# jspenmar/slowtv_monodepth

Measured on AMD Instinct MI355X. Metric: training images/sec (640×192, 3-frame) at 1/2/4/8 MI355X; warp+SSIM HBM GB/s, higher is better.
Workload: dtype f32

## Files before the change

include/smd_hotpath.h:

```cpp
#ifndef SMD_HOTPATH_H
#define SMD_HOTPATH_H

#include <stddef.h>
#include <stdint.h>

#ifdef __cplusplus
extern "C" {
#endif

#define SMD_ABI_VERSION 8

#define SMD_OK 0
#define SMD_E_INVALID (-1)
#define SMD_E_LAUNCH (-2)
#define SMD_E_WORKSPACE (-3)
#define SMD_E_UNSUPPORTED (-4)

#define SMD_USE_MIN 0x1
#define SMD_USE_AUTOMASK 0x2
#define SMD_LOSS_L1 0x4
#define SMD_NEED_K_GRAD 0x8
#define SMD_USE_EDGES 0x10
#define SMD_LOSS_L2 0x20
#define SMD_MASK_EXPLAINABILITY 0x80
// ... 151 lines not shown
int smd_conv3x3_mfma_fwd(const void* xp, const void* wp_fwd, void* y, void* workspace, size_t workspace_bytes,
                         int B, int C, int CO, int h, int w, int pieces, void* stream);
int smd_conv3x3_mfma_bwd_data(const void* g_y, const void* wp_bwd, void* g_xp, void* workspace, size_t workspace_bytes,
                              int B, int C, int CO, int h, int w, int pieces, void* stream);
int smd_conv3x3_mfma_bwd_weight(const void* xp, const void* g_y, float* g_weight, void* workspace, size_t workspace_bytes,
                                int B, int C, int CO, int h, int w, int pieces, void* stream);

size_t smd_conv3x3z_mfma_workspace_bytes(int B, int C, int CO, int h, int w);
int smd_conv3x3z_mfma_fwd(const float* x, const void* wp_fwd, float* y, void* workspace, size_t workspace_bytes,
                          int B, int C, int CO, int h, int w, int pieces, void* stream);
int smd_conv3x3z_mfma_bwd_data(const float* g_y, const void* wp_bwd, float* g_x, void* workspace, size_t workspace_bytes,
                               int B, int C, int CO, int h, int w, int pieces, void* stream);
int smd_conv3x3z_mfma_bwd_weight(const float* x, const float* g_y, float* g_weight, void* workspace, size_t workspace_bytes,
                                 int B, int C, int CO, int h, int w, int pieces, void* stream);

size_t smd_conv7x7s2_packed_bytes(int C, int CO);
size_t smd_conv7x7s2_workspace_bytes(int B, int C, int CO, int H, int W);
int smd_conv7x7s2_pack(const float* weight, void* wp, int C, int CO, void* stream);
int smd_conv7x7s2_fwd(const float* x, const void* wp, float* y, int B, int C, int CO, int H, int W, void* stream);
int smd_conv7x7s2_bwd_weight(const float* x, const float* g_y, float* g_weight, void* workspace, size_t workspace_bytes,
                             int B, int C, int CO, int H, int W, void* stream);

size_t smd_bn_workspace_bytes(int N, int C, int HW);
int smd_bn_fwd(const float* x, const float* residual, const float* gamma, const float* beta, float* running_mean, float* running_var,
               float momentum, float eps, int relu, float* y, float* save_mean, float* save_invstd,
               void* workspace, size_t workspace_bytes, int N, int C, int HW, void* stream);
int smd_bn_bwd(const float* x, const float* y, const float* g_y, const float* gamma, const float* save_mean, const float* save_invstd,
               int relu, float* g_x, float* g_residual, float* g_gamma, float* g_beta,
               void* workspace, size_t workspace_bytes, int N, int C, int HW, void* stream);

// ... 98 lines not shown
```

slowtv_monodepth_amd/_lib.py:

```python
from __future__ import annotations

import ctypes as C
import os
from pathlib import Path

import torch

__all__ = ['lib', 'call', 'set_knob', 'reset_knobs', 'knob_epoch', 'lib_path', 'FLAGS', 'REGR_FLAGS', 'SEL_MASKED', 'ptr_array', 'int_array', 'i64_array', 'HotpathError', 'Unsupported']

_HERE = Path(__file__).resolve().parent
lib_path = Path(os.environ.get('SMD_HOTPATH_LIB', _HERE/'libsmd_hotpath.so'))

FLAGS = {'use_min': 0x1, 'use_automask': 0x2, 'loss_l1': 0x4, 'need_k_grad': 0x8, 'use_edges': 0x10, 'loss_l2': 0x20, 'packed_ready': 0x40,
         'mask_explainability': 0x80, 'mask_uncertainty': 0x100, 'use_laplacian': 0x200, 'bwd_skip_rows': 0x400, 'edges_ready': 0x800, 'bwd_no_live': 0x1000}
REGR_FLAGS = {'l1': 0x0, 'log_l1': 0x1, 'berhu': 0x2, 'invert': 0x4}
SEL_MASKED = 255
MAX_SCALES = 8
MAX_SUPPORTS = 8

_vp, _i, _f, _sz, _u64 = C.c_void_p, C.c_int, C.c_float, C.c_size_t, C.c_uint64

PROTOTYPES = {
    'smd_last_error': (C.c_char_p, []),
    'smd_abi_version': (_i, []),
# ... 46 lines not shown
    'smd_scale_mean_fwd': (_i, [_vp]*2 + [_i]*2 + [_vp]*2 + [_sz, _vp]),
    'smd_scale_mean_bwd': (_i, [_vp]*2 + [_i]*2 + [_vp]*3),
    'smd_conv3x3_thin_workspace_bytes': (_sz, [_i]*4),
    'smd_conv3x3_thin_fwd': (_i, [_vp]*3 + [_i]*4 + [_vp]),
    'smd_conv3x3_thin_bwd': (_i, [_vp]*6 + [_sz] + [_i]*4 + [_vp]),
    'smd_conv3x3_mfma_packed_bytes': (_sz, [_i]*3),
    'smd_conv3x3_mfma_workspace_bytes': (_sz, [_i]*5),
    'smd_conv3x3_mfma_pack': (_i, [_vp]*3 + [_i]*3 + [_vp]),
    'smd_conv3x3_mfma_fwd': (_i, [_vp]*4 + [_sz] + [_i]*6 + [_vp]),
    'smd_conv3x3_mfma_bwd_data': (_i, [_vp]*4 + [_sz] + [_i]*6 + [_vp]),
    'smd_conv3x3_mfma_bwd_weight': (_i, [_vp]*4 + [_sz] + [_i]*6 + [_vp]),
    'smd_conv3x3z_mfma_workspace_bytes': (_sz, [_i]*5),
    'smd_conv3x3z_mfma_fwd': (_i, [_vp]*4 + [_sz] + [_i]*6 + [_vp]),
    'smd_conv3x3z_mfma_bwd_data': (_i, [_vp]*4 + [_sz] + [_i]*6 + [_vp]),
    'smd_conv3x3z_mfma_bwd_weight': (_i, [_vp]*4 + [_sz] + [_i]*6 + [_vp]),
    'smd_conv7x7s2_packed_bytes': (_sz, [_i]*2),
    'smd_conv7x7s2_workspace_bytes': (_sz, [_i]*5),
    'smd_conv7x7s2_pack': (_i, [_vp]*2 + [_i]*2 + [_vp]),
    'smd_conv7x7s2_fwd': (_i, [_vp]*3 + [_i]*5 + [_vp]),
    'smd_conv7x7s2_bwd_weight': (_i, [_vp]*4 + [_sz] + [_i]*5 + [_vp]),
    'smd_conv3x3_head_workspace_bytes': (_sz, [_i]*4),
    'smd_conv3x3_head_fwd': (_i, [_vp]*4 + [_i]*5 + [_vp]),
    'smd_conv3x3_head_bwd': (_i, [_vp]*8 + [_sz] + [_i]*5 + [_vp]),
    'smd_elu_pad_fwd': (_i, [_vp]*3 + [_i]*6 + [_vp]),
    'smd_elu_pad_bwd': (_i, [_vp]*6 + [_sz] + [_i]*6 + [_vp]),
    'smd_elu_up_cat_pad_fwd': (_i, [_vp]*4 + [_i]*6 + [_vp]),
    'smd_elu_up_cat_pad_bwd': (_i, [_vp]*7 + [_sz] + [_i]*6 + [_vp]),
    'smd_bn_workspace_bytes': (_sz, [_i, _i, _i]),
    'smd_bn_fwd': (_i, [_vp]*6 + [_f, _f, _i] + [_vp]*4 + [_sz] + [_i]*3 + [_vp]),
    'smd_bn_bwd': (_i, [_vp]*6 + [_i] + [_vp]*5 + [_sz] + [_i]*3 + [_vp]),
# ... 102 lines not shown
```

slowtv_monodepth_amd/conv_ops.py:

```python
from __future__ import annotations

from collections import namedtuple

import torch

from . import _lib
from ._device import _check, _check_fb, _on, _ptr, _stream, _workspace, call
from .conv_routing import serve

_BF = torch.bfloat16


def _thin_bwd(xp, weight, g_y, want_x, want_w):
    if not (want_x or want_w): return None, None
    B, C, H, W = xp.shape
    g_xp = torch.empty_like(xp) if want_x else None
    g_w = torch.empty_like(weight) if want_w else None
    ws, nbytes = _workspace(xp.device, _lib.lib.smd_conv3x3_thin_workspace_bytes, B, C, H - 2, W - 2, floor=256) if want_w else (None, 0)
    call('smd_conv3x3_thin_bwd', xp.data_ptr(), weight.data_ptr(), g_y.data_ptr(), _ptr(g_xp), _ptr(g_w), _ptr(ws), nbytes, B, C, H - 2, W - 2, _stream())
    return g_xp, g_w


class _Conv3x3Thin(torch.autograd.Function):
    @staticmethod
# ... 38 lines not shown
    return wf, wb


def _mfma_ws_bytes(B, C, CO, h, w, zpad):
    return (_lib.lib.smd_conv3x3z_mfma_workspace_bytes if zpad else _lib.lib.smd_conv3x3_mfma_workspace_bytes)(B, C, CO, h, w)


def _mfma_launch(entry, zpad, a, b, out, nws, dims, pieces):
    ws, nws = _workspace(out.device, nws, floor=256)
    call(('smd_conv3x3z_mfma_' if zpad else 'smd_conv3x3_mfma_') + entry, a.data_ptr(), b.data_ptr(), out.data_ptr(), ws.data_ptr(), nws, *dims, pieces, _stream())
    return out


class _Conv3x3Wide(torch.autograd.Function):
    @staticmethod
    def forward(ctx, xp, weight, pieces, force, zpad=False):
        xp = _check_fb('xp', xp)
        if zpad and xp.dtype != torch.float32: raise TypeError(f'the zero-padded convolution takes float32 tensors, got {xp.dtype}')
        if xp.ndim != 4 or (not zpad and (xp.shape[2] < 3 or xp.shape[3] < 3)):
            raise ValueError(f'expected {"(B,C,h,w)" if zpad else "a padded (B,C,h+2,w+2)"}, got {tuple(xp.shape)}')
        B, C, H, W = xp.shape
        if weight.ndim != 4 or tuple(weight.shape[1:]) != (C, 3, 3): raise ValueError(f'weight: expected (CO,{C},3,3), got {tuple(weight.shape)}')
        CO = weight.shape[0]
        weight = _check('weight', weight, (CO, C, 3, 3))
        h, w = (H, W) if zpad else (H - 2, W - 2)
        dims = (B, C, CO, h, w)
        bf = xp.dtype == _BF
        if bf: pieces = 1
        nws = _mfma_ws_bytes(*dims, zpad)
        sv = _served(C, CO, zpad, force or nws > 0)
        if force and not sv.fwd:
# ... 6 lines not shown
            return _mfma_launch('fwd', zpad, xp, packed['wf'], y, nws, dims, pieces)

        def run_ref():
            if zpad: return torch.conv2d(xp, weight, None, 1, 1)
            if bf: return torch.conv2d(xp, weight.to(_BF))
            if sv.thin: call('smd_conv3x3_thin_fwd', xp.data_ptr(), weight.data_ptr(), y.data_ptr(), B, C, h, w, _stream()); return y
            return torch.conv2d(xp, weight)
        op = 'fwd_z' if zpad else 'fwd_bf16' if bf else 'fwd'
        out = serve((op, *dims), run_mfma, run_ref, eligible=sv.fwd and sv.sized, force=force)
        ctx.save_for_backward(xp, weight, packed.get('wb'))
        ctx.pieces, ctx.force, ctx.zpad, ctx.served = pieces, force, zpad, sv
        return out

    @staticmethod
    def backward(ctx, g_y):
        xp, weight, wp_bwd = ctx.saved_tensors
        return (*_wide_backward(xp, weight, wp_bwd, g_y, ctx.pieces, ctx.force, ctx.zpad, ctx.served, *ctx.needs_input_grad[:2]), None, None, None)


def _wide_backward(xp, weight, wp_bwd, g_y, pieces, force, zpad, sv, need_x, need_w, deterministic_ref=False):
    _on(xp)
    B, C, H, W = xp.shape
    CO = weight.shape[0]
    h, w = (H, W) if zpad else (H - 2, W - 2)
    dims = (B, C, CO, h, w)
    bf = xp.dtype == _BF
    g_y = _check_fb('grad(y)', g_y.to(xp.dtype), (B, CO, h, w))
    g_xp = g_w = None
    w_ref = weight.to(_BF) if bf else weight
    pad = [1, 1] if zpad else [0, 0]
    def cb(mask):
        det = torch.backends.cudnn.deterministic
# ... 20 lines not shown
    return g_xp, g_w


def conv3x3_mfma(xp, weight, pieces: int = 3):
    return _Conv3x3Wide.apply(xp, weight, int(pieces), True)


def conv3x3_wide(xp, weight):
    return _Conv3x3Wide.apply(xp, weight, 3, False)


def conv3x3_same(x, weight):
    return _Conv3x3Wide.apply(x, weight, 3, False, True)


class _Conv7x7s2Stem(torch.autograd.Function):
    @staticmethod
    def forward(ctx, x, weight):
        x = _check('x', x)
        if x.ndim != 4: raise ValueError(f'expected (B,C,H,W), got {tuple(x.shape)}')
        B, C, H, W = x.shape
        if weight.ndim != 4 or tuple(weight.shape[1:]) != (C, 7, 7): raise ValueError(f'weight: expected (CO,{C},7,7), got {tuple(weight.shape)}')
        CO = weight.shape[0]
        weight = _check('weight', weight, (CO, C, 7, 7))
        ho, wo = (H - 1)//2 + 1, (W - 1)//2 + 1
        served = _lib.lib.smd_conv7x7s2_workspace_bytes(B, C, CO, H, W) > 0
        y = torch.empty((B, CO, ho, wo), device=x.device, dtype=torch.float32)

        def run_mfma():
            wp, _ = _workspace(x.device, _lib.lib.smd_conv7x7s2_packed_bytes, C, CO)
# ... 33 lines not shown
```

slowtv_monodepth_amd/conv_routing.py:

```python
from __future__ import annotations

import torch

from ._lib import Unsupported

_MODE = 'auto'
_ROUTES: dict = {}
_AB_WARMUPS, _AB_ROUNDS, _AB_MARGIN = 2, 5, 0.97
_DECLINED = (Unsupported, ValueError)


def set_conv_route(mode: str = 'auto'):
    global _MODE
    if mode not in ('auto', 'mfma', 'miopen'): raise ValueError(mode)
    _MODE = mode
    _ROUTES.clear()


def conv_routes() -> dict:
    return dict(_ROUTES)


_COARSE_W_MAX, _COARSE_C_MIN = 80, 256
_Z_FWD_WGT = [dict(px_min=1000, ch_max=511), dict(px_min=2400)]
# ... 3 lines not shown
               'wgt': [dict(thin=False, px_min=20000, co_max=64), dict(thin=False, coarse=True, px_min=2400)]},
    'bf16': {'fwd': [dict(thin=True)], 'data': [dict(thin=True)], 'wgt': [dict(thin=True)]},
    'zpad': {'fwd': _Z_FWD_WGT, 'data': [dict(px_min=1000)], 'wgt': _Z_FWD_WGT},
    'stem': {'fwd': [dict(px_min=20000)], 'wgt': [dict(px_min=20000)]},
}
_FAMILY_OF_SUFFIX = {'': 'padded', 'bf16': 'bf16', 'z': 'zpad', 's': 'stem'}
_BOUNDS = {'px_min': lambda v, B, C, CO, h, w: B*h*w >= v,
           'c_max': lambda v, B, C, CO, h, w: C <= v,
           'co_max': lambda v, B, C, CO, h, w: CO <= v,
           'c_co_max': lambda v, B, C, CO, h, w: C*CO <= v,
           'ch_max': lambda v, B, C, CO, h, w: max(C, CO) <= v,
           'thin': lambda v, B, C, CO, h, w: (CO == 16) == v,
           'coarse': lambda v, B, C, CO, h, w: (w <= _COARSE_W_MAX and C >= _COARSE_C_MIN) == v}


def static_rule(op, B, C, CO, h, w) -> bool:
    kind, _, suffix = op.partition('_')
    clauses = STATIC_RULES[_FAMILY_OF_SUFFIX[suffix]][kind]
    return any(all(_BOUNDS[name](v, B, C, CO, h, w) for name, v in clause.items()) for clause in clauses)


_capturing = torch.cuda.is_current_stream_capturing


def _time_interleaved(run_mfma, run_ref, rounds):
    ev = [[torch.cuda.Event(enable_timing=True) for _ in range(3)] for _ in range(rounds)]
    for e in ev:
        e[0].record(); run_mfma(); e[1].record(); run_ref(); e[2].record()
    torch.cuda.synchronize()
    return [e[0].elapsed_time(e[1])*1e3 for e in ev], [e[1].elapsed_time(e[2])*1e3 for e in ev]


def _conv_route(op, B, C, CO, h, w, run_mfma, run_ref) -> bool:
    if _MODE != 'auto': return _MODE == 'mfma'
# ... 26 lines not shown
```

slowtv_monodepth_amd/csrc/smd_api.hip:

```cpp
#include <limits.h>
#include <math.h>
#include <stdarg.h>
#include <stdio.h>
#include <stdlib.h>
#include <string.h>
#include <algorithm>

#include "smd_kernels.h"
#include "smd_smooth_dev.h"

namespace {

thread_local char g_err[512] = "";

int fail(int code, const char* fmt, ...) {
  va_list ap;
  va_start(ap, fmt);
  vsnprintf(g_err, sizeof(g_err), fmt, ap);
  va_end(ap);
  return code;
}

int check_launch(hipError_t e, const char* what) {
  if (e != hipSuccess) return fail(SMD_E_LAUNCH, "%s: %s", what, hipGetErrorString(e));
// ... 880 lines not shown
int smd_conv3x3_mfma_bwd_data(const void* g_y, const void* wp_bwd, void* g_xp, void* workspace, size_t workspace_bytes, int B, int C, int CO, int h, int w, int pieces, void* stream) {
  return mfma_form(ConvOp::Data, false, g_y, wp_bwd, g_xp, workspace, workspace_bytes, B, C, CO, h, w, pieces, stream, "conv3x3_mfma_bwd_data");
}
int smd_conv3x3_mfma_bwd_weight(const void* xp, const void* g_y, float* g_weight, void* workspace, size_t workspace_bytes, int B, int C, int CO, int h, int w, int pieces, void* stream) {
  return mfma_bwd_weight(false, xp, g_y, g_weight, workspace, workspace_bytes, B, C, CO, h, w, pieces, stream);
}
int smd_conv3x3z_mfma_fwd(const float* x, const void* wp_fwd, float* y, void* workspace, size_t workspace_bytes, int B, int C, int CO, int h, int w, int pieces, void* stream) {
  return mfma_form(ConvOp::Fwd, true, x, wp_fwd, y, workspace, workspace_bytes, B, C, CO, h, w, pieces, stream, "conv3x3z_mfma_fwd");
}
int smd_conv3x3z_mfma_bwd_data(const float* g_y, const void* wp_bwd, float* g_x, void* workspace, size_t workspace_bytes, int B, int C, int CO, int h, int w, int pieces, void* stream) {
  return mfma_form(ConvOp::Data, true, g_y, wp_bwd, g_x, workspace, workspace_bytes, B, C, CO, h, w, pieces, stream, "conv3x3z_mfma_bwd_data");
}
int smd_conv3x3z_mfma_bwd_weight(const float* x, const float* g_y, float* g_weight, void* workspace, size_t workspace_bytes, int B, int C, int CO, int h, int w, int pieces, void* stream) {
  return mfma_bwd_weight(true, x, g_y, g_weight, workspace, workspace_bytes, B, C, CO, h, w, pieces, stream);
}
static bool stem_sizes_ok(int B, int C, int H, int W) {
  if (B < 1 || B > 65535 || C < 1 || H < 1 || W < 1) return false;
  const long long ho = (H - 1)/2 + 1, wo = (W - 1)/2 + 1;
  return (long long)C*H*W < (1ll << 31) && 64*ho*wo < (1ll << 31) && (ho + 3)/4 <= 65535;
}
size_t smd_conv7x7s2_packed_bytes(int C, int CO) { return smd::conv_stem_served(C, CO) ? smd::conv_stem_packed_bytes(C) : 0; }
size_t smd_conv7x7s2_workspace_bytes(int B, int C, int CO, int H, int W) {
  if (!smd::conv_stem_served(C, CO) || !stem_sizes_ok(B, C, H, W)) return 0;
  return align256(smd::conv_stem_wgrad_floats(B, C, H, W)*sizeof(float));
}
int smd_conv7x7s2_pack(const float* weight, void* wp, int C, int CO, void* stream) {
  if (!weight || !wp) return fail(SMD_E_INVALID, "null pointer");
  if (!smd::conv_stem_served(C, CO)) return fail(SMD_E_UNSUPPORTED, "the stem kernels serve CO == 64 with C == 3 | 6, not C=%d CO=%d", C, CO);
  return check_launch(smd::launch_conv_stem_pack(weight, wp, C, (hipStream_t)stream), "conv7x7s2_pack");
}
// ... 406 lines not shown
```

slowtv_monodepth_amd/csrc/smd_conv_mfma.hip:

```cpp
#include "smd_common.h"
#include "smd_kernels.h"
#include "smd_conv_mfma_dev.h"
#include <algorithm>

namespace smd {

template <typename T> __device__ __forceinline__ void store_out(T* p, size_t i, float v);
template <> __device__ __forceinline__ void store_out<float>(float* p, size_t i, float v) { p[i] = v; }
template <> __device__ __forceinline__ void store_out<bf16>(bf16* p, size_t i, float v) { p[i] = __float2bfloat16(v); }

template <int P>
__global__ __launch_bounds__(256) void k_conv_pack_w(const float* __restrict__ w, unsigned short* __restrict__ wp_fwd, unsigned short* __restrict__ wp_bwd, int CO, int C) {
  const int idx = blockIdx.x*256 + threadIdx.x;
  if (idx >= CO*C*9) return;
  const int tap = idx % 9, c = (idx/9) % C, co = idx/(9*C);
  unsigned pk[P];
  split_pair<P>(w[idx], 0.f, pk);
  if (wp_fwd) {
    const size_t base = ((((size_t)(co >> 5)*(C >> 4) + (c >> 4))*9 + tap)*P)*512 + (((c >> 3) & 1)*32 + (co & 31))*8 + (c & 7);
#pragma unroll
    for (int p = 0; p < P; ++p) wp_fwd[base + (size_t)p*512] = (unsigned short)(pk[p] & 0xffffu);
  }
  if (wp_bwd) {
    const size_t base = ((((size_t)(c >> 5)*(CO >> 4) + (co >> 4))*9 + (8 - tap))*P)*512 + (((co >> 3) & 1)*32 + (c & 31))*8 + (co & 7);
// ... 284 lines not shown
    }
  }
}

template <typename TO>
__global__ __launch_bounds__(256) void k_conv_split_sum(const float* __restrict__ part, TO* __restrict__ out, size_t n4, int KS) {
  const size_t i = (size_t)blockIdx.x*256 + threadIdx.x;
  if (i >= n4) return;
  const f4* p = reinterpret_cast<const f4*>(part);
  f4 s = p[i];
  for (int k = 1; k < KS; ++k) s += p[(size_t)k*n4 + i];
  if constexpr (sizeof(TO) == 4) reinterpret_cast<f4*>(out)[i] = s;
  else { unsigned* o = reinterpret_cast<unsigned*>(out) + 2*i; o[0] = pack_bf16_rne(s.x, s.y); o[1] = pack_bf16_rne(s.z, s.w); }
}

static size_t thin_packed_elems(int C, int pieces) { return (size_t)(C >> 4)*5*pieces*512; }
size_t conv_mfma_packed_elems(int C, int CO, int pieces) { return std::max((size_t)CO*C*9*pieces, CO == 16 ? thin_packed_elems(C, pieces) : (size_t)0); }

#define SMD_BY_PIECES(pieces, CALL) do { if ((pieces) == 3) { CALL(3, float); } else if ((pieces) == 2) { CALL(2, float); } else { CALL(1, bf16); } } while (0)

template <int P, typename T>
static void launch_conv16(const void* in, const void* wp, void* out, int B, int CK, bool bwd, int hi, int wi, int ho, int wo, hipStream_t st) {
  const unsigned gx = ceil_div(wo, 64), gy = ceil_div(ho, 4), gz = B;
  const dim3 grid(8*(unsigned)ceil_div((long long)gx*gy*gz, 8ll));
  const uint4* wq = (const uint4*)wp;
  const T* i_ = (const T*)in; T* o_ = (T*)out;
  if (bwd) hipLaunchKernelGGL((k_conv16_mfma<1, P, true, T, T>), grid, dim3(256), 0, st, i_, wq, o_, hi, wi, ho, wo, gx, gy, gz);
  else if (CK == 16) hipLaunchKernelGGL((k_conv16_mfma<1, P, false, T, T>), grid, dim3(256), 0, st, i_, wq, o_, hi, wi, ho, wo, gx, gy, gz);
  else hipLaunchKernelGGL((k_conv16_mfma<2, P, false, T, T>), grid, dim3(256), 0, st, i_, wq, o_, hi, wi, ho, wo, gx, gy, gz);
}
// ... 137 lines not shown
```

slowtv_monodepth_amd/csrc/smd_kernels.h:

```cpp
#pragma once
#include <hip/hip_runtime.h>
#include <stddef.h>
#include <stdint.h>

#include "../../include/smd_hotpath.h"

namespace smd {

constexpr int kFwdCols = 62;
constexpr int kBwdCols = 60;
#ifndef SMD_WAVES_PER_BLOCK
#define SMD_WAVES_PER_BLOCK 4
#endif
constexpr int kWavesPerBlock = SMD_WAVES_PER_BLOCK;
#ifndef SMD_SMOOTH_CHUNK
#define SMD_SMOOTH_CHUNK 1024
#endif
constexpr int kSmoothChunk = SMD_SMOOTH_CHUNK;
__host__ __device__ inline int smooth_chunk_px(int n) { return n > 32768 ? kSmoothChunk : 256; }
__host__ __device__ inline int smooth_chunks_of(int n) { return (n + smooth_chunk_px(n) - 1)/smooth_chunk_px(n); }
constexpr int kSmoothCols = 63, kSmoothRows = 8;
__host__ __device__ inline int smooth_units_of(int hs, int ws) { return ((ws + kSmoothCols - 1)/kSmoothCols)*((hs + kSmoothRows - 1)/kSmoothRows); }
constexpr int kSmoothRowsMain = 16;
__host__ __device__ inline int smooth_units_main(int hs, int ws) { return ((ws + kSmoothCols - 1)/kSmoothCols)*((hs + kSmoothRowsMain - 1)/kSmoothRowsMain); }
// ... 209 lines not shown
hipError_t launch_conv_thin_bwd_data(const float* gy, const float* wgt, float* g_xp, int B, int C, int h, int w, hipStream_t st);
enum class ConvOp { Fwd, Data, Wgt };
inline bool conv_mfma_served(ConvOp op, bool zpad, int C, int CO) {
  const bool thin = !zpad && CO == 16 && (C == 16 || C == 32);
  if (op == ConvOp::Fwd) return (C % 16 == 0 && CO % 32 == 0) || thin;
  if (op == ConvOp::Data) return (CO % 16 == 0 && C % 32 == 0) || (thin && C == 16);
  return CO % 32 == 0 || thin;
}
size_t conv_mfma_packed_elems(int C, int CO, int pieces);
size_t conv_mfma_wgrad_partials(bool zpad, int B, int C, int CO, int h, int w);
size_t conv_mfma_split_elems(ConvOp op, bool zpad, int B, int C, int CO, int h, int w, bool two_tiles);
hipError_t launch_conv_mfma_pack(const float* w, void* wp_fwd, void* wp_bwd, int C, int CO, int pieces, hipStream_t st);
hipError_t launch_conv_mfma_fwd(const void* x, const void* wp_fwd, void* y, float* split_ws, bool zpad, int B, int C, int CO, int h, int w, int pieces, bool two_tiles, hipStream_t st);
hipError_t launch_conv_mfma_bwd_data(const void* gy, const void* wp_bwd, void* g_x, float* split_ws, bool zpad, int B, int C, int CO, int h, int w, int pieces, bool two_tiles, hipStream_t st);
hipError_t launch_conv_mfma_bwd_wgt(const void* x, const void* gy, float* g_w, float* partial, bool zpad, int B, int C, int CO, int h, int w, int pieces, hipStream_t st);
struct SetIndexMap { int CO = 0, C = 0; };
size_t partial_sets_floats(unsigned T, size_t n);
hipError_t launch_partial_sets_finalize(float* partial, unsigned T, int n, SetIndexMap index_map, float* g_w, hipStream_t st);
bool conv_stem_served(int C, int CO);
size_t conv_stem_packed_bytes(int C);
size_t conv_stem_wgrad_floats(int B, int C, int H, int W);
hipError_t launch_conv_stem_pack(const float* w, void* wp, int C, hipStream_t st);
hipError_t launch_conv_stem_fwd(const float* x, const void* wp, float* y, int B, int C, int H, int W, hipStream_t st);
hipError_t launch_conv_stem_bwd_wgt(const float* x, const float* gy, float* g_w, float* partial, int B, int C, int H, int W, hipStream_t st);
size_t decoder_bias_partials(int B, int C, int h, int w);
hipError_t launch_elu_pad_fwd(const void* x, const float* bias, void* out, int B, int C, int h, int w, int apply_elu, int dt, hipStream_t st);
hipError_t launch_elu_pad_bwd(const void* x, const float* bias, const void* g_out, void* g_x, float* g_bias, float* ws, int B, int C, int h, int w,
                              int apply_elu, int dt, hipStream_t st);
hipError_t launch_elu_up_cat_pad_fwd(const void* a, const float* bias, const void* skip, void* out, int B, int Ca, int Cs, int h, int w, int dt,
                                     hipStream_t st);
// ... 112 lines not shown
```

slowtv_monodepth_amd/functional.py:

```python
from ._device import _stream, call
from .attention_ops import channel_attention, se_gate
from .blend import flip_blend, flip_blend_pyramid
from .ddv_ops import ddv_head
from .fusion_ops import relu_pad, up_cat_gate_pad
from .class_ops import _ScaleMean, crop_resize, lane_shift_selftest, photo_error, recon_reduce, regression_loss, scale_mean, upsample_stack, view_synth
from .conv_ops import conv3x3_mfma, conv3x3_same, conv3x3_thin, conv3x3_wide, conv7x7s2_stem
from .conv_routing import _conv_route, conv_routes, set_conv_route
from .geom_ops import intrinsics, inv_intrinsics, pose_matrices
from .metric_ops import depth_metrics
from .net_ops import batch_norm_act, conv3x3_head, conv3x3_headn, dwconv7x7, elu_pad, elu_up_cat_pad, layer_norm_cf, max_pool3x3s2
from .recon_ops import (PreparedFrames, disp_smooth_blurred, disp_smooth_fused, disp_to_depth, gaussian_blur3x3, image_recon_fused, image_recon_fused_disp,
                        image_recon_prep, loss_path_fused, recon_flags, supports_per_pass)
from .row_skip import _RowSkipTuner, dead_tile_shares, dead_wave_shares, row_skip_tuner
from .subpixel import subpixel_conv

__all__ = ['conv3x3_headn', 'upsample_stack', 'scale_mean', 'conv3x3_mfma', 'conv3x3_wide', 'conv3x3_same', 'set_conv_route', 'conv_routes', 'loss_path_fused', 'crop_resize', 'disp_to_depth', 'image_recon_prep', 'PreparedFrames', 'image_recon_fused', 'image_recon_fused_disp', 'disp_smooth_fused', 'view_synth', 'photo_error', 'recon_reduce',
           'lane_shift_selftest', 'recon_flags', 'regression_loss', 'elu_pad', 'elu_up_cat_pad', 'batch_norm_act', 'max_pool3x3s2', 'dwconv7x7', 'layer_norm_cf', 'pose_matrices', 'intrinsics', 'inv_intrinsics',
           'conv3x3_head', 'conv3x3_thin', 'conv7x7s2_stem', 'gaussian_blur3x3', 'disp_smooth_blurred', 'supports_per_pass', 'row_skip_tuner', 'dead_tile_shares', 'dead_wave_shares', 'depth_metrics']
```

slowtv_monodepth_amd/networks/encoders.py:

```python
from __future__ import annotations

import torch
import torch.nn as nn
import torch.nn.functional as F

__all__ = ['create_encoder', 'FeatureInfo', 'ResNetFeatures', 'ConvNeXtFeatures', 'ENCODERS']


class FeatureInfo:
    def __init__(self, channels, reduction): self._c, self._r = list(channels), list(reduction)
    def channels(self): return list(self._c)
    def reduction(self): return list(self._r)


class BatchNormAct2d(nn.BatchNorm2d):
    fused_enabled = True

    def forward(self, x, residual=None, relu: bool = False):
        fused = (self.fused_enabled and x.is_cuda and self.training and x.dtype == torch.float32 and not torch.is_autocast_enabled() and self.affine
                 and self.track_running_stats and self.momentum is not None and x.is_contiguous())
        if not fused:
            y = super().forward(x)
            if residual is not None: y = y + residual
            return F.relu(y, inplace=True) if relu else y
# ... 5 lines not shown
    def flush_counter(self):
        n = getattr(self, '_pending_batches', 0)
        if n and self.num_batches_tracked is not None: self.num_batches_tracked += n
        self._pending_batches = 0

    def _save_to_state_dict(self, destination, prefix, keep_vars):
        self.flush_counter()
        super()._save_to_state_dict(destination, prefix, keep_vars)

    def train(self, mode: bool = True):
        if not mode: self.flush_counter()
        return super().train(mode)


def _conv3x3(conv: nn.Conv2d, x):
    if (conv.stride == (1, 1) and BatchNormAct2d.fused_enabled and x.is_cuda and x.dtype == torch.float32 and conv.weight.dtype == torch.float32
            and not torch.is_autocast_enabled() and x.is_contiguous()):
        from .. import functional as HF
        return HF.conv3x3_same(x, conv.weight)
    return conv(x)


def _stem(conv: nn.Conv2d, x):
    if (BatchNormAct2d.fused_enabled and x.is_cuda and x.dtype == torch.float32 and conv.weight.dtype == torch.float32
            and not torch.is_autocast_enabled() and x.is_contiguous()):
        from .. import functional as HF
        return HF.conv7x7s2_stem(x, conv.weight)
    return conv(x)


class BasicBlock(nn.Module):
    def __init__(self, cin, cout, stride):
        super().__init__()
        self.conv1 = nn.Conv2d(cin, cout, 3, stride, 1, bias=False); self.bn1 = BatchNormAct2d(cout)
# ... 143 lines not shown
```

Measured before the change: 958.1.

## Add MFMA stride-2 3x3 conv kernels for encoder downsampling layers

Adds a new HIP kernel that runs stride-2 3x3 convolutions (forward and data gradient) on MFMA using split bf16 pieces. It decomposes each conv by output or input phase parity into tap subsets and can split the K dimension across blocks with a reduction. The encoder now routes stride-2 convs through it, gated by static shape rules and an eligibility check, and falls back to torch otherwise. The aim is to replace the vendor library for the downsampling convs in ResNet blocks; the weight gradient still uses the torch path, and the bf16 split could slightly change numerics.

```diff
diff --git a/include/smd_hotpath.h b/include/smd_hotpath.h
--- a/include/smd_hotpath.h
+++ b/include/smd_hotpath.h
@@ -189,6 +189,12 @@
 int smd_conv3x3z_mfma_bwd_weight(const float* x, const float* g_y, float* g_weight, void* workspace, size_t workspace_bytes,
                                  int B, int C, int CO, int h, int w, int pieces, void* stream);
 
+size_t smd_conv3x3s2_mfma_workspace_bytes(int B, int C, int CO, int H, int W);
+int smd_conv3x3s2_mfma_fwd(const float* x, const void* wp_fwd, float* y, void* workspace, size_t workspace_bytes,
+                           int B, int C, int CO, int H, int W, int pieces, void* stream);
+int smd_conv3x3s2_mfma_bwd_data(const float* g_y, const void* wp_bwd, float* g_x, void* workspace, size_t workspace_bytes,
+                                int B, int C, int CO, int H, int W, int pieces, void* stream);
+
 size_t smd_conv7x7s2_packed_bytes(int C, int CO);
 size_t smd_conv7x7s2_workspace_bytes(int B, int C, int CO, int H, int W);
 int smd_conv7x7s2_pack(const float* weight, void* wp, int C, int CO, void* stream);
diff --git a/slowtv_monodepth_amd/_lib.py b/slowtv_monodepth_amd/_lib.py
--- a/slowtv_monodepth_amd/_lib.py
+++ b/slowtv_monodepth_amd/_lib.py
@@ -84,6 +84,9 @@
     'smd_conv3x3z_mfma_fwd': (_i, [_vp]*4 + [_sz] + [_i]*6 + [_vp]),
     'smd_conv3x3z_mfma_bwd_data': (_i, [_vp]*4 + [_sz] + [_i]*6 + [_vp]),
     'smd_conv3x3z_mfma_bwd_weight': (_i, [_vp]*4 + [_sz] + [_i]*6 + [_vp]),
+    'smd_conv3x3s2_mfma_workspace_bytes': (_sz, [_i]*5),
+    'smd_conv3x3s2_mfma_fwd': (_i, [_vp]*4 + [_sz] + [_i]*6 + [_vp]),
+    'smd_conv3x3s2_mfma_bwd_data': (_i, [_vp]*4 + [_sz] + [_i]*6 + [_vp]),
     'smd_conv7x7s2_packed_bytes': (_sz, [_i]*2),
     'smd_conv7x7s2_workspace_bytes': (_sz, [_i]*5),
     'smd_conv7x7s2_pack': (_i, [_vp]*2 + [_i]*2 + [_vp]),
diff --git a/slowtv_monodepth_amd/conv_ops.py b/slowtv_monodepth_amd/conv_ops.py
--- a/slowtv_monodepth_amd/conv_ops.py
+++ b/slowtv_monodepth_amd/conv_ops.py
@@ -76,7 +76,9 @@
 
 class _Conv3x3Wide(torch.autograd.Function):
     @staticmethod
-    def forward(ctx, xp, weight, pieces, force, zpad=False):
+    def forward(ctx, xp, weight, pieces, force, zpad=False, stride=1):
+        ctx.stride = stride
+        if stride == 2: return _s2_forward(ctx, xp, weight)
         xp = _check_fb('xp', xp)
         if zpad and xp.dtype != torch.float32: raise TypeError(f'the zero-padded convolution takes float32 tensors, got {xp.dtype}')
         if xp.ndim != 4 or (not zpad and (xp.shape[2] < 3 or xp.shape[3] < 3)):
@@ -113,8 +115,9 @@
 
     @staticmethod
     def backward(ctx, g_y):
+        if ctx.stride == 2: return (*_s2_backward(ctx, g_y), None, None, None, None)
         xp, weight, wp_bwd = ctx.saved_tensors
-        return (*_wide_backward(xp, weight, wp_bwd, g_y, ctx.pieces, ctx.force, ctx.zpad, ctx.served, *ctx.needs_input_grad[:2]), None, None, None)
+        return (*_wide_backward(xp, weight, wp_bwd, g_y, ctx.pieces, ctx.force, ctx.zpad, ctx.served, *ctx.needs_input_grad[:2]), None, None, None, None)
 
 
 def _wide_backward(xp, weight, wp_bwd, g_y, pieces, force, zpad, sv, need_x, need_w, deterministic_ref=False):
@@ -165,6 +168,64 @@
     return _Conv3x3Wide.apply(x, weight, 3, False, True)
 
 
+def _s2_forward(ctx, x, weight):
+    for name, t in (('x', x), ('weight', weight)):
+        if not isinstance(t, torch.Tensor): raise TypeError(f'{name} must be a Tensor, got {type(t)}')
+        if t.dtype != torch.float32: raise TypeError(f'{name} must be float32, got {t.dtype}')
+    if x.ndim != 4: raise ValueError(f'expected (B,C,H,W), got {tuple(x.shape)}')
+    B, C, H, W = x.shape
+    if weight.ndim != 4 or tuple(weight.shape[1:]) != (C, 3, 3): raise ValueError(f'weight: expected (CO,{C},3,3), got {tuple(weight.shape)}')
+    x = _check('x', x)
+    CO = weight.shape[0]
+    weight = _check('weight', weight, (CO, C, 3, 3))
+    dims = (B, C, CO, H, W)
+    nws = _lib.lib.smd_conv3x3s2_mfma_workspace_bytes(*dims)
+    data_ok = nws > 0 and C % 32 == 0
+    y = torch.empty((B, CO, (H - 1)//2 + 1, (W - 1)//2 + 1), device=x.device, dtype=torch.float32)
+    packed = {}
+
+    def run_mfma():
+        packed['wf'], packed['wb'] = _mfma_pack(weight, C, CO, 3, True, data_ok)
+        return _s2_launch('fwd', x, packed['wf'], y, nws, dims)
+    out = serve(('fwd_z2', *dims), run_mfma, lambda: torch.conv2d(x, weight, None, 2, 1), eligible=nws > 0)
+    ctx.save_for_backward(x, weight, packed.get('wb'))
+    ctx.nws, ctx.data_ok = nws, data_ok
+    return out
+
+
+def _s2_backward(ctx, g_y):
+    x, weight, wp_bwd = ctx.saved_tensors
+    _on(x)
+    B, C, H, W = x.shape
+    CO = weight.shape[0]
+    dims = (B, C, CO, H, W)
+    need_x, need_w = ctx.needs_input_grad[:2]
+    g_y = _check('grad(y)', g_y, (B, CO, (H - 1)//2 + 1, (W - 1)//2 + 1))
+    cb = lambda mask: torch.ops.aten.convolution_backward(g_y, x, weight, None, [2, 2], [1, 1], [1, 1], False, [0, 0], 1, mask)
+    g_x = g_w = None
+    if need_x:
+        g_x = torch.empty_like(x)
+        packed = {'wb': wp_bwd}
+
+        def run_data():
+            if packed['wb'] is None: packed['wb'] = _mfma_pack(weight, C, CO, 3, False, True)[1]
+            return _s2_launch('bwd_data', g_y, packed['wb'], g_x, ctx.nws, dims)
+        g_x = serve(('data_z2', *dims), run_data, lambda: cb([True, False, False])[0], eligible=ctx.data_ok)
+    if need_w:
+        g_w = serve(('wgt_z2', *dims), None, lambda: cb([False, True, False])[1], eligible=False)
+    return g_x, g_w
+
+
+def _s2_launch(entry, a, b, out, nws, dims):
+    ws, nws = _workspace(out.device, nws, floor=256)
+    call('smd_conv3x3s2_mfma_' + entry, a.data_ptr(), b.data_ptr(), out.data_ptr(), ws.data_ptr(), nws, *dims, 3, _stream())
+    return out
+
+
+def conv3x3_s2(x, weight):
+    return _Conv3x3Wide.apply(x, weight, 3, False, True, 2)
+
+
 class _Conv7x7s2Stem(torch.autograd.Function):
     @staticmethod
     def forward(ctx, x, weight):
diff --git a/slowtv_monodepth_amd/conv_routing.py b/slowtv_monodepth_amd/conv_routing.py
--- a/slowtv_monodepth_amd/conv_routing.py
+++ b/slowtv_monodepth_amd/conv_routing.py
@@ -41,10 +41,22 @@
            'coarse': lambda v, B, C, CO, h, w: (w <= _COARSE_W_MAX and C >= _COARSE_C_MIN) == v}
 
 
+def _meets(clauses, B, C, CO, h, w) -> bool:
+    return any(all(_BOUNDS[name](v, B, C, CO, h, w) for name, v in clause.items()) for clause in clauses)
+
+
+S2_STATIC_RULE = {'fwd': [dict(c_max=64, px_min=90000)], 'data': [dict(c_max=128, px_min=23000)], 'wgt': []}
+
+
+def static_rule_s2(kind, B, C, CO, h, w) -> bool:
+    if C % 16 or CO % 32 or (kind == 'data' and C % 32): return False
+    return _meets(S2_STATIC_RULE[kind], B, C, CO, h, w)
+
+
 def static_rule(op, B, C, CO, h, w) -> bool:
     kind, _, suffix = op.partition('_')
-    clauses = STATIC_RULES[_FAMILY_OF_SUFFIX[suffix]][kind]
-    return any(all(_BOUNDS[name](v, B, C, CO, h, w) for name, v in clause.items()) for clause in clauses)
+    if suffix == 'z2': return static_rule_s2(kind, B, C, CO, h, w)
+    return _meets(STATIC_RULES[_FAMILY_OF_SUFFIX[suffix]][kind], B, C, CO, h, w)
 
 
 _capturing = torch.cuda.is_current_stream_capturing
diff --git a/slowtv_monodepth_amd/csrc/smd_api.hip b/slowtv_monodepth_amd/csrc/smd_api.hip
--- a/slowtv_monodepth_amd/csrc/smd_api.hip
+++ b/slowtv_monodepth_amd/csrc/smd_api.hip
@@ -918,6 +918,29 @@
 int smd_conv3x3z_mfma_bwd_weight(const float* x, const float* g_y, float* g_weight, void* workspace, size_t workspace_bytes, int B, int C, int CO, int h, int w, int pieces, void* stream) {
   return mfma_bwd_weight(true, x, g_y, g_weight, workspace, workspace_bytes, B, C, CO, h, w, pieces, stream);
 }
+static bool s2_sizes_ok(int B, int C, int CO, int H, int W) {
+  return mfma_sizes_ok(B, C, CO, H, W) && smd::conv_s2_blocks(ConvOp::Fwd, B, C, CO, H, W) < (1ll << 30) && smd::conv_s2_blocks(ConvOp::Data, B, C, CO, H, W) < (1ll << 30);
+}
+size_t smd_conv3x3s2_mfma_workspace_bytes(int B, int C, int CO, int H, int W) {
+  if (!smd::conv_s2_served(ConvOp::Fwd, C, CO) || !s2_sizes_ok(B, C, CO, H, W)) return 0;
+  return align256(std::max({(size_t)64, smd::conv_s2_split_elems(ConvOp::Fwd, B, C, CO, H, W), smd::conv_s2_split_elems(ConvOp::Data, B, C, CO, H, W)})*sizeof(float));
+}
+static int s2_form(ConvOp op, const float* in, const void* wp, float* out, void* workspace, size_t workspace_bytes, int B, int C, int CO, int H, int W, int pieces, void* stream, const char* what) {
+  if (!in || !wp || !out || !workspace) return fail(SMD_E_INVALID, "null pointer");
+  if (pieces != 3) return fail(SMD_E_UNSUPPORTED, "the stride-2 forms take float tensors split into 3 pieces, not %d", pieces);
+  if (!s2_sizes_ok(B, C, CO, H, W)) return fail(SMD_E_INVALID, "invalid sizes B=%d C=%d CO=%d H=%d W=%d", B, C, CO, H, W);
+  if (!smd::conv_s2_served(ConvOp::Fwd, C, CO) || !smd::conv_s2_served(op, C, CO))
+    return fail(SMD_E_UNSUPPORTED, "the stride-2 %s does not serve C=%d CO=%d", op == ConvOp::Fwd ? "forward" : "data gradient", C, CO);
+  if (workspace_bytes < smd_conv3x3s2_mfma_workspace_bytes(B, C, CO, H, W)) return fail(SMD_E_WORKSPACE, "workspace too small");
+  const auto launch = op == ConvOp::Fwd ? smd::launch_conv_s2_fwd : smd::launch_conv_s2_bwd_data;
+  return check_launch(launch(in, wp, out, (float*)workspace, B, C, CO, H, W, (hipStream_t)stream), what);
+}
+int smd_conv3x3s2_mfma_fwd(const float* x, const void* wp_fwd, float* y, void* workspace, size_t workspace_bytes, int B, int C, int CO, int H, int W, int pieces, void* stream) {
+  return s2_form(ConvOp::Fwd, x, wp_fwd, y, workspace, workspace_bytes, B, C, CO, H, W, pieces, stream, "conv3x3s2_mfma_fwd");
+}
+int smd_conv3x3s2_mfma_bwd_data(const float* g_y, const void* wp_bwd, float* g_x, void* workspace, size_t workspace_bytes, int B, int C, int CO, int H, int W, int pieces, void* stream) {
+  return s2_form(ConvOp::Data, g_y, wp_bwd, g_x, workspace, workspace_bytes, B, C, CO, H, W, pieces, stream, "conv3x3s2_mfma_bwd_data");
+}
 static bool stem_sizes_ok(int B, int C, int H, int W) {
   if (B < 1 || B > 65535 || C < 1 || H < 1 || W < 1) return false;
   const long long ho = (H - 1)/2 + 1, wo = (W - 1)/2 + 1;
diff --git a/slowtv_monodepth_amd/csrc/smd_conv_mfma.hip b/slowtv_monodepth_amd/csrc/smd_conv_mfma.hip
--- a/slowtv_monodepth_amd/csrc/smd_conv_mfma.hip
+++ b/slowtv_monodepth_amd/csrc/smd_conv_mfma.hip
@@ -322,6 +322,11 @@
   else { unsigned* o = reinterpret_cast<unsigned*>(out) + 2*i; o[0] = pack_bf16_rne(s.x, s.y); o[1] = pack_bf16_rne(s.z, s.w); }
 }
 
+hipError_t launch_conv_split_sum(const float* part, float* out, size_t n4, int KS, hipStream_t st) {
+  hipLaunchKernelGGL((k_conv_split_sum<float>), dim3((unsigned)((n4 + 255)/256)), dim3(256), 0, st, part, out, n4, KS);
+  return hipGetLastError();
+}
+
 static size_t thin_packed_elems(int C, int pieces) { return (size_t)(C >> 4)*5*pieces*512; }
 size_t conv_mfma_packed_elems(int C, int CO, int pieces) { return std::max((size_t)CO*C*9*pieces, CO == 16 ? thin_packed_elems(C, pieces) : (size_t)0); }
 
diff --git a/slowtv_monodepth_amd/csrc/smd_conv_s2.hip b/slowtv_monodepth_amd/csrc/smd_conv_s2.hip
--- /dev/null
+++ b/slowtv_monodepth_amd/csrc/smd_conv_s2.hip
@@ -0,0 +1,204 @@
+#include "smd_common.h"
+#include "smd_kernels.h"
+#include "smd_conv_mfma_dev.h"
+#include <algorithm>
+#include <type_traits>
+
+namespace smd {
+
+template <int TC> struct S2Tile {
+  static constexpr int TRB = (TC == 64) ? 4 : 8;
+  static constexpr int PW = TC + 1, PH = TRB + 1, NPIX = PW*PH;
+};
+
+template <int PQ, bool DATA> struct S2Taps {
+  static constexpr int p = PQ >> 1, q = PQ & 1, NX = q ? 2 : 1, N = (p ? 2 : 1)*NX;
+  static constexpr int ky(int t) { return p ? 2*(t/NX) : 1; }
+  static constexpr int kx(int t) { return q ? 2*(t % NX) : 1; }
+  static constexpr int dr(int t) { return DATA ? (p ? (2 - ky(t))/2 : 0) : (p ? ky(t)/2 : 1); }
+  static constexpr int dc(int t) { return DATA ? (q ? (2 - kx(t))/2 : 0) : (q ? kx(t)/2 : 1); }
+  static constexpr int widx(int t) { return DATA ? 8 - (3*ky(t) + kx(t)) : 3*ky(t) + kx(t); }
+};
+
+template <int TC, int P, bool DATA>
+__global__ __launch_bounds__(256, 2) void k_conv_s2_mfma(const float* __restrict__ in_, const uint4* __restrict__ wp, float* __restrict__ out,
+                                                         int CK, int M, int hi, int wi, int ho, int wo, int KS, int kc_per_split, size_t split_stride,
+                                                         unsigned gx, unsigned gy, unsigned gz) {
+  using T = S2Tile<TC>;
+  constexpr int NPIX = T::NPIX, PW = T::PW, TRB = T::TRB;
+  using Stage = PatchStager<256, NPIX, P, float, true>;
+  constexpr int TRIPS = Stage::TRIPS, NST = DATA ? 1 : 4;
+  __shared__ uint4 tile[2*Stage::kBuf];
+  const int lane = threadIdx.x & 63, wv = __builtin_amdgcn_readfirstlane(threadIdx.x >> 6), j = lane & 31, g = lane >> 5;
+  const int MG = M/32;
+  const unsigned nblk = (unsigned)(MG*KS)*(DATA ? 4u : 1u)*gx*gy*gz, lid = xcd_block_id(nblk);
+  if (lid >= nblk) return;
+  const int mg = (int)(lid % MG), ks = (int)((lid/MG) % KS);
+  unsigned tl = lid/(MG*KS);
+  const int ph = DATA ? (int)(tl & 3u) : 0;
+  if (DATA) tl >>= 2;
+  const int x0 = (int)(tl % gx)*TC, y0 = (int)((tl/gx) % gy)*TRB, b = (int)(tl/(gx*gy));
+  const int KC = CK >> 4, kc0 = ks*kc_per_split, kc1 = min(KC, kc0 + kc_per_split);
+  const size_t plane = (size_t)hi*wi;
+  const float* src = in_ + (size_t)b*CK*plane;
+
+  Stage stage[NST];
+#pragma unroll
+  for (int s = 0; s < NST; ++s) {
+    const int p = DATA ? ph >> 1 : s >> 1, q = DATA ? ph & 1 : s & 1;
+#pragma unroll
+    for (int t = 0; t < TRIPS; ++t) {
+      const int it = Stage::item(t), half = it >= NPIX ? 1 : 0, pix = it - half*NPIX;
+      const int r = pix/PW, cc = pix - r*PW;
+      int yy, xx;
+      bool used;
+      if (DATA) { yy = y0 + r; xx = x0 + cc; used = (p || r < TRB) && (q || cc < TC); }
+      else { yy = 2*(y0 - 1 + r) + p; xx = 2*(x0 - 1 + cc) + q; used = (p || r > 0) && (q || cc > 0); }
+      stage[s].pofs[t] = (used && yy >= 0 && yy < hi && xx >= 0 && xx < wi) ? yy*wi + xx : -1;
+    }
+  }
+  float v[TRIPS][8];
+  f32x16 acc[2], lo[2];
+#pragma unroll
+  for (int nt = 0; nt < 2; ++nt)
+#pragma unroll
+    for (int r = 0; r < 16; ++r) { acc[nt][r] = 0.f; lo[nt][r] = 0.f; }
+
+  bf16x8 A[4][P];
+  const uint4* wq = wp + ((size_t)mg*KC*9*P)*64 + lane;
+  auto fetch_a = [&](auto taps, int kc) __attribute__((always_inline)) {
+    using TP = decltype(taps);
+#pragma unroll
+    for (int t = 0; t < TP::N; ++t)
+#pragma unroll
+      for (int p = 0; p < P; ++p) A[t][p] = as_frag(wq[(size_t)((kc*9 + TP::widx(t))*P + p)*64]);
+  };
+  auto read_b = [&](bf16x8 (&dst)[2][P], int buf, int dr, int dc) __attribute__((always_inline)) {
+#pragma unroll
+    for (int nt = 0; nt < 2; ++nt) {
+      const int r = (TC == 64) ? wv : 2*wv + nt, cb = (TC == 64) ? nt*32 : 0;
+      Stage::read(tile, buf, (r + dr)*PW + cb + j + dc, g, dst[nt]);
+    }
+  };
+  auto mma = [&](auto taps, int buf) __attribute__((always_inline)) {
+    using TP = decltype(taps);
+    bf16x8 Bf[2][2][P];
+    read_b(Bf[0], buf, TP::dr(0), TP::dc(0));
+#pragma unroll
+    for (int t = 0; t < TP::N; ++t) {
+      if (t + 1 < TP::N) read_b(Bf[(t + 1) & 1], buf, TP::dr(t + 1), TP::dc(t + 1));
+      split_mfma<P>(A[t], Bf[t & 1], acc, lo);
+    }
+  };
+  auto step = [&](auto taps, int cur, auto next_taps, auto next_stage_idx, int next_kc, auto next_tag) __attribute__((always_inline)) {
+    constexpr bool NEXT = decltype(next_tag)::value;
+    const Stage& next_stage = stage[decltype(next_stage_idx)::value];
+    if constexpr (NEXT) next_stage.request(src, plane, next_kc, v);
+    mma(taps, cur);
+    if constexpr (NEXT) { fetch_a(next_taps, next_kc); next_stage.file(tile, cur ^ 1, v); }
+    __syncthreads();
+  };
+
+  if constexpr (!DATA) {
+    using T0 = S2Taps<0, false>; using T1 = S2Taps<1, false>; using T2 = S2Taps<2, false>; using T3 = S2Taps<3, false>;
+    auto chunk = [&](int kc, auto more) __attribute__((always_inline)) {
+      step(T0{}, 0, T1{}, std::integral_constant<int, 1>{}, kc, std::true_type{});
+      step(T1{}, 1, T2{}, std::integral_constant<int, 2>{}, kc, std::true_type{});
+      step(T2{}, 0, T3{}, std::integral_constant<int, 3>{}, kc, std::true_type{});
+      step(T3{}, 1, T0{}, std::integral_constant<int, 0>{}, kc + 1, more);
+    };
+    if (kc0 < kc1) {
+      stage[0].request(src, plane, kc0, v);
+      fetch_a(T0{}, kc0);
+      stage[0].file(tile, 0, v);
+    }
+    __syncthreads();
+    int kc = kc0;
+    for (; kc + 1 < kc1; ++kc) chunk(kc, std::true_type{});
+    if (kc < kc1) chunk(kc, std::false_type{});
+  } else {
+    auto run = [&](auto taps) __attribute__((always_inline)) {
+      if (kc0 < kc1) {
+        stage[0].request(src, plane, kc0, v);
+        fetch_a(taps, kc0);
+        stage[0].file(tile, 0, v);
+      }
+      __syncthreads();
+      int kc = kc0;
+      for (; kc + 1 < kc1; ++kc) step(taps, (kc - kc0) & 1, taps, std::integral_constant<int, 0>{}, kc + 1, std::true_type{});
+      if (kc < kc1) step(taps, (kc - kc0) & 1, taps, std::integral_constant<int, 0>{}, kc, std::false_type{});
+    };
+    if (ph == 0) run(S2Taps<0, true>{});
+    else if (ph == 1) run(S2Taps<1, true>{});
+    else if (ph == 2) run(S2Taps<2, true>{});
+    else run(S2Taps<3, true>{});
+  }
+
+  float* dst = out + (size_t)ks*split_stride;
+#pragma unroll
+  for (int nt = 0; nt < 2; ++nt) {
+    const int r = (TC == 64) ? wv : 2*wv + nt, cb = (TC == 64) ? nt*32 : 0;
+    const int y = DATA ? 2*(y0 + r) + (ph >> 1) : y0 + r, x = DATA ? 2*(x0 + cb + j) + (ph & 1) : x0 + cb + j;
+    if (y < ho && x < wo) {
+#pragma unroll
+      for (int rr = 0; rr < 16; ++rr) {
+        const int m = mg*32 + mfma32_row(rr, g);
+        dst[(((size_t)b*M + m)*ho + y)*wo + x] = acc[nt][rr] + lo[nt][rr];
+      }
+    }
+  }
+}
+
+bool conv_s2_served(ConvOp op, int C, int CO) {
+  if (op == ConvOp::Fwd) return C % 16 == 0 && CO % 32 == 0;
+  if (op == ConvOp::Data) return CO % 16 == 0 && C % 32 == 0;
+  return false;
+}
+namespace {
+struct S2Shape { int TC, KS, kcs; unsigned gx, gy, gz; long long blocks; size_t out_elems; };
+S2Shape s2_shape(bool data, int B, int CK, int M, int th, int tw, size_t out_elems) {
+  S2Shape s;
+  const long long t64 = (long long)ceil_div(tw, 64)*ceil_div(th, 4), t32 = (long long)ceil_div(tw, 32)*ceil_div(th, 8);
+  s.TC = t32 < t64 ? 32 : 64;
+  s.gx = ceil_div(tw, s.TC); s.gy = ceil_div(th, s.TC == 64 ? 4 : 8); s.gz = B;
+  const int KC = CK >> 4;
+  const long long base = (long long)s.gx*s.gy*s.gz*(data ? 4 : 1)*(M/32);
+  int ks = 1;
+  if (base < 384) ks = (int)std::min<long long>(std::max(KC/2, 1), (512 + base - 1)/base);
+  s.kcs = ceil_div(KC, ks); s.KS = ceil_div(KC, s.kcs);
+  s.blocks = base*s.KS;
+  s.out_elems = out_elems;
+  return s;
+}
+S2Shape s2_shape_of(ConvOp op, int B, int C, int CO, int H, int W) {
+  const int ho = (H - 1)/2 + 1, wo = (W - 1)/2 + 1;
+  return op == ConvOp::Fwd ? s2_shape(false, B, C, CO, ho, wo, (size_t)B*CO*ho*wo) : s2_shape(true, B, CO, C, ho, wo, (size_t)B*C*H*W);
+}
+}
+long long conv_s2_blocks(ConvOp op, int B, int C, int CO, int H, int W) { return conv_s2_served(op, C, CO) ? s2_shape_of(op, B, C, CO, H, W).blocks : 0; }
+size_t conv_s2_split_elems(ConvOp op, int B, int C, int CO, int H, int W) {
+  if (!conv_s2_served(op, C, CO)) return 0;
+  const S2Shape s = s2_shape_of(op, B, C, CO, H, W);
+  return s.KS > 1 ? (size_t)s.KS*s.out_elems : 0;
+}
+
+template <bool DATA>
+static hipError_t launch_s2(const float* in, const void* wp, float* out, float* split_ws, const S2Shape& s, int CK, int M, int hi, int wi, int ho, int wo, hipStream_t st) {
+  const dim3 grid(8*(unsigned)ceil_div(s.blocks, 8ll));
+  float* dst = s.KS > 1 ? split_ws : out;
+  const uint4* wq = (const uint4*)wp;
+  if (s.TC == 64) hipLaunchKernelGGL((k_conv_s2_mfma<64, 3, DATA>), grid, dim3(256), 0, st, in, wq, dst, CK, M, hi, wi, ho, wo, s.KS, s.kcs, s.out_elems, s.gx, s.gy, s.gz);
+  else hipLaunchKernelGGL((k_conv_s2_mfma<32, 3, DATA>), grid, dim3(256), 0, st, in, wq, dst, CK, M, hi, wi, ho, wo, s.KS, s.kcs, s.out_elems, s.gx, s.gy, s.gz);
+  if (s.KS > 1) return launch_conv_split_sum(split_ws, out, s.out_elems/4, s.KS, st);
+  return hipGetLastError();
+}
+hipError_t launch_conv_s2_fwd(const float* x, const void* wp_fwd, float* y, float* split_ws, int B, int C, int CO, int H, int W, hipStream_t st) {
+  const int ho = (H - 1)/2 + 1, wo = (W - 1)/2 + 1;
+  return launch_s2<false>(x, wp_fwd, y, split_ws, s2_shape_of(ConvOp::Fwd, B, C, CO, H, W), C, CO, H, W, ho, wo, st);
+}
+hipError_t launch_conv_s2_bwd_data(const float* gy, const void* wp_bwd, float* g_x, float* split_ws, int B, int C, int CO, int H, int W, hipStream_t st) {
+  const int ho = (H - 1)/2 + 1, wo = (W - 1)/2 + 1;
+  return launch_s2<true>(gy, wp_bwd, g_x, split_ws, s2_shape_of(ConvOp::Data, B, C, CO, H, W), CO, C, ho, wo, H, W, st);
+}
+
+}
diff --git a/slowtv_monodepth_amd/csrc/smd_kernels.h b/slowtv_monodepth_amd/csrc/smd_kernels.h
--- a/slowtv_monodepth_amd/csrc/smd_kernels.h
+++ b/slowtv_monodepth_amd/csrc/smd_kernels.h
@@ -247,6 +247,12 @@
 hipError_t launch_conv_mfma_fwd(const void* x, const void* wp_fwd, void* y, float* split_ws, bool zpad, int B, int C, int CO, int h, int w, int pieces, bool two_tiles, hipStream_t st);
 hipError_t launch_conv_mfma_bwd_data(const void* gy, const void* wp_bwd, void* g_x, float* split_ws, bool zpad, int B, int C, int CO, int h, int w, int pieces, bool two_tiles, hipStream_t st);
 hipError_t launch_conv_mfma_bwd_wgt(const void* x, const void* gy, float* g_w, float* partial, bool zpad, int B, int C, int CO, int h, int w, int pieces, hipStream_t st);
+hipError_t launch_conv_split_sum(const float* part, float* out, size_t n4, int KS, hipStream_t st);
+bool conv_s2_served(ConvOp op, int C, int CO);
+long long conv_s2_blocks(ConvOp op, int B, int C, int CO, int H, int W);
+size_t conv_s2_split_elems(ConvOp op, int B, int C, int CO, int H, int W);
+hipError_t launch_conv_s2_fwd(const float* x, const void* wp_fwd, float* y, float* split_ws, int B, int C, int CO, int H, int W, hipStream_t st);
+hipError_t launch_conv_s2_bwd_data(const float* gy, const void* wp_bwd, float* g_x, float* split_ws, int B, int C, int CO, int H, int W, hipStream_t st);
 struct SetIndexMap { int CO = 0, C = 0; };
 size_t partial_sets_floats(unsigned T, size_t n);
 hipError_t launch_partial_sets_finalize(float* partial, unsigned T, int n, SetIndexMap index_map, float* g_w, hipStream_t st);
diff --git a/slowtv_monodepth_amd/functional.py b/slowtv_monodepth_amd/functional.py
--- a/slowtv_monodepth_amd/functional.py
+++ b/slowtv_monodepth_amd/functional.py
@@ -4,7 +4,7 @@
 from .ddv_ops import ddv_head
 from .fusion_ops import relu_pad, up_cat_gate_pad
 from .class_ops import _ScaleMean, crop_resize, lane_shift_selftest, photo_error, recon_reduce, regression_loss, scale_mean, upsample_stack, view_synth
-from .conv_ops import conv3x3_mfma, conv3x3_same, conv3x3_thin, conv3x3_wide, conv7x7s2_stem
+from .conv_ops import conv3x3_mfma, conv3x3_s2, conv3x3_same, conv3x3_thin, conv3x3_wide, conv7x7s2_stem
 from .conv_routing import _conv_route, conv_routes, set_conv_route
 from .geom_ops import intrinsics, inv_intrinsics, pose_matrices
 from .metric_ops import depth_metrics
diff --git a/slowtv_monodepth_amd/networks/encoders.py b/slowtv_monodepth_amd/networks/encoders.py
--- a/slowtv_monodepth_amd/networks/encoders.py
+++ b/slowtv_monodepth_amd/networks/encoders.py
@@ -43,10 +43,10 @@
 
 
 def _conv3x3(conv: nn.Conv2d, x):
-    if (conv.stride == (1, 1) and BatchNormAct2d.fused_enabled and x.is_cuda and x.dtype == torch.float32 and conv.weight.dtype == torch.float32
+    if (conv.stride in ((1, 1), (2, 2)) and BatchNormAct2d.fused_enabled and x.is_cuda and x.dtype == torch.float32 and conv.weight.dtype == torch.float32
             and not torch.is_autocast_enabled() and x.is_contiguous()):
         from .. import functional as HF
-        return HF.conv3x3_same(x, conv.weight)
+        return (HF.conv3x3_same if conv.stride == (1, 1) else HF.conv3x3_s2)(x, conv.weight)
     return conv(x)
 
 
```

After: 961.6 (median of 3 runs). About the same (+0.4%).
